# TrackieWay-OSS/TrackieLLM

Hardware: AMD Instinct MI355X
Metric: cortex cycles/sec (frame+1s audio+128 tok) (higher is better)
Workload: dtype int8 x q4_K/q6_K (i32 acc, f32 scales); 1 GPU; configs[3] fused cycle: YOLOv8n 640x640 frame (preprocess+network+NMS) + 1 s PCM (VAD + Whisper-tiny.en log-mel/encoder/16 forced decoder steps) + Mistral-7B Q4_K_M 64-token prefill and 128-token greedy decode, 3 concurrent HIP streams; concurrent_cycles_per_gpu=768, decode_groups=3, rows_per_llm_pass=256, layers=32, parallelism=replicas x1

## Files before the change

### include/tk/tk_mi355x_ext.h

```cpp
#ifndef TK_MI355X_EXT_H
#define TK_MI355X_EXT_H

#include "tk_types.h"

#ifdef __cplusplus
extern "C" {
#endif

typedef struct {
    int32_t n_layer, d_model, n_head, n_kv_head, head_dim, d_ff, vocab;
    float rms_eps, rope_theta;
    int32_t ks_qkv, ks_o, ks_gateup, ks_down, ks_out;
} tk_mi355x_llm_hparams_t;

typedef struct tk_mi355x_llm_model_s tk_mi355x_llm_model_t;
typedef struct tk_mi355x_llm_session_s tk_mi355x_llm_session_t;

TK_API const char* tk_mi355x_version(void);
TK_API int tk_mi355x_device_count(void);
TK_API void tk_mi355x_set_default_device(int device);
TK_API int tk_mi355x_get_default_device(void);

TK_API TK_NODISCARD tk_error_code_t tk_mi355x_llm_model_create(tk_mi355x_llm_model_t** out, const tk_mi355x_llm_hparams_t* hp, int device);
TK_API TK_NODISCARD tk_error_code_t tk_mi355x_llm_model_fill_synthetic(tk_mi355x_llm_model_t* m, uint64_t seed);
// ... 137 lines not shown

TK_API TK_NODISCARD tk_error_code_t tk_mi355x_llm_time_attention(tk_mi355x_llm_session_t* s, int nrows, int ctx, int iters, float* avg_ms,
                                                                 double* kv_bytes);

TK_API int tk_mi355x_device_cu_count(int device);
TK_API TK_NODISCARD tk_error_code_t tk_mi355x_attention_plan(int device, int nrows, int n_head, int n_kv_head, int head_dim, int max_ctx, int fused, int32_t out[4]);
TK_API TK_NODISCARD tk_error_code_t tk_mi355x_attention_plan_at(int device, int nrows, int n_head, int n_kv_head, int head_dim, int max_ctx, int fused,
                                                                int top_position, int32_t out[4]);
TK_API TK_NODISCARD tk_error_code_t tk_mi355x_attention_plan_verify(int device, int nrows, int n_head, int n_kv_head, int head_dim, int max_ctx,
                                                                    int top_position, int32_t out[4]);

TK_API TK_NODISCARD tk_error_code_t tk_mi355x_grammar_check(const char* gbnf, const char* text, int32_t* n_accepted, int32_t* complete);
TK_API TK_NODISCARD tk_error_code_t tk_mi355x_grammar_next_bytes(const char* gbnf, const char* prefix, uint8_t allowed[256], int32_t* complete);
struct tk_llm_runner_s;
TK_API const char* tk_mi355x_llm_runner_tool_call_text(struct tk_llm_runner_s* runner);

TK_API TK_NODISCARD tk_error_code_t tk_mi355x_gemm_pair(int device, int M, int N, int K, const float* a, const float* w, const float* bias,
                                                        const float* residual, int act, int f16, float* c_staged, float* c_tiled);

typedef struct {
    int32_t M, N, K, lda, ldb, ldc, ldr, b_kn, act;
    float alpha;
    int32_t batch, batch_inner;
    int64_t sA, sB, sC, sR, sA2, sB2, sC2, sR2;
    int32_t b_f16;
    int32_t im_C, im_H, im_W, im_ldx, im_kw, im_stride, im_pad, im_Ho, im_Wo;
    int32_t fast;
    int32_t a_offset, b_offset;
    int32_t kernel;
    const float* a; const void* b; const float* bias; const float* residual; float* c;
    int64_t n_a, n_b, n_bias, n_residual, n_c;
} tk_mi355x_gemm_probe_t;
TK_API TK_NODISCARD tk_error_code_t tk_mi355x_gemm_probe(int device, tk_mi355x_gemm_probe_t* p);

TK_API TK_NODISCARD tk_error_code_t tk_mi355x_attention_h3_probe(int device, int B, int nh, int Tq, int Tk, int64_t q_bstride, int64_t kv_bstride, int d, float scale,
                                                                 const float* q, const float* k, const float* v, int64_t n_q, int64_t n_kv, float* out);

enum { TK_MI355X_PICK_ARGMAX = 0, TK_MI355X_PICK_ARGMAX_ROWS = 1, TK_MI355X_PICK_ROWS = 2, TK_MI355X_PICK_ROWS_FILTERED = 3 };
typedef struct {
    int32_t kind, rows, cols, ld;
    const float* logits;
    int64_t n_logits;
    const uint32_t* masks;
    const int32_t* allow_row;
    int32_t n_masks, hist_stride;
    tk_mi355x_sampling_t* samp;
    int32_t *tok, *pos, *nsteps, *hist;
    int64_t n_hist;
    float temperature;
    uint32_t counter0;
    uint64_t seed;
    float* logprob;
    const uint8_t* suppress;
    int32_t* state;
    int32_t beg, eot, tid0, reserved;
} tk_mi355x_token_pick_probe_t;
TK_API TK_NODISCARD tk_error_code_t tk_mi355x_token_pick_probe(int device, tk_mi355x_token_pick_probe_t* p);

TK_API TK_NODISCARD tk_error_code_t tk_mi355x_logit_adjust_probe(int device, int32_t rows, int32_t cols, float* logits, int64_t n_logits,
                                                                 const tk_mi355x_logit_adjust_t* adjust);

TK_API TK_NODISCARD tk_error_code_t tk_mi355x_lang_pick_probe(int device, int32_t rows, int32_t cols, int32_t ld, const float* logits, int64_t n_logits, int32_t tok0,
                                                              int32_t n_lang, const int32_t* auto_row, int32_t* slot, int32_t* ids, float* probs);

enum {
    TK_MI355X_STEP_EMBED = 0, TK_MI355X_STEP_RMSNORM = 1, TK_MI355X_STEP_RESIDUAL_FOLD = 2, TK_MI355X_STEP_SWIGLU = 3, TK_MI355X_STEP_QUANT = 4,
// ... 111 lines not shown
```

### trackiellm_amd/csrc/hal/tk_rocm_hal.hip

```cpp
#include <hip/hip_runtime.h>
#include <math.h>
#include <stdlib.h>

#include <vector>

#include "../common/tk_exact_math.h"
#include "../common/tk_lang_pick.h"
#include "tk/tk_mi355x_ext.h"

#include "../vision/tk_vision_engine.h"
#include "../vision/tk_depth_engine.h"
#include "../audio/tk_audio_engine.h"
#include "tk/tk_rocm_hal.h"
#include "../nn/tk_gemm_tiled.h"
#include "../nn/tk_nn_kernels.h"
#include "../llm/tk_llm_kernels.h"

struct tk_gpu_buffer_s {
    void* dptr;
    size_t size;
};

struct tk_rocm_dispatcher_s {
    int device;
    hipStream_t compute, h2d, d2h;
    hipEvent_t ev_upload, ev_compute;
};

__global__ void k_postprocess_depth(tk_postprocess_depth_params_t p) {
    const size_t n = (size_t)p.width * p.height;
    for (size_t i = (size_t)blockIdx.x * blockDim.x + threadIdx.x; i < n; i += (size_t)gridDim.x * blockDim.x)
        p.d_metric_depth_map[i] = p.d_raw_depth_map[i] * p.scale + p.shift;
}

__global__ void k_depth_to_points(tk_depth_to_points_params_t p) {
    const size_t n = (size_t)p.width * p.height;
    for (size_t i = (size_t)blockIdx.x * blockDim.x + threadIdx.x; i < n; i += (size_t)gridDim.x * blockDim.x) {
        const float d = p.d_metric_depth_map[i];
        tk_float3 o = {0.0f, 0.0f, 0.0f};
        if (d > 0.0f) {
            const float u = (float)(i % p.width), v = (float)(i / p.width);
            o.x = tk_divf((u - p.cx) * d, p.fx);
            o.y = tk_divf((v - p.cy) * d, p.fy);
            o.z = d;
        }
        p.d_point_cloud[i] = o;
    }
// ... 135 lines not shown
    return ok ? TK_SUCCESS : TK_ERROR_GPU_ROCM_ERROR;
}

struct ProbeReach { int64_t a, b, c, r; };
static bool probe_reach(const tk_mi355x_gemm_probe_t& p, ProbeReach& o) {
    const int64_t cap = (int64_t)1 << 28;
    auto dim = [&](int64_t v) { return v >= 1 && v <= cap; };
    auto str = [&](int64_t v) { return v >= 0 && v <= cap; };
    if (!dim(p.M) || !dim(p.N) || !dim(p.K) || !dim(p.ldb) || !dim(p.ldc) || p.ldc < p.N || p.act < 0 || p.act > 3) return false;
    if (p.batch < 1 || p.batch > 4096 || p.batch_inner < 0 || p.batch_inner > p.batch || (p.batch_inner > 0 && p.batch % p.batch_inner)) return false;
    if ((p.b_kn != 0 && p.b_kn != 1) || (p.b_f16 != 0 && p.b_f16 != 1) || p.a_offset < 0 || p.a_offset > 64 || p.b_offset < 0 || p.b_offset > 64) return false;
    const int64_t st[8] = {p.sA, p.sB, p.sC, p.sR, p.sA2, p.sB2, p.sC2, p.sR2};
    for (int64_t v : st) if (!str(v)) return false;
    if (p.residual && (!dim(p.ldr) || p.ldr < p.N)) return false;
    const int64_t zi = p.batch_inner > 0 ? p.batch_inner - 1 : p.batch - 1, zo = p.batch_inner > 0 ? p.batch / p.batch_inner - 1 : 0;
    auto last = [&](int64_t s1, int64_t s2) { return zi * s1 + (p.batch_inner > 0 ? zo * s2 : 0); };
    if (p.im_C > 0) {
        if (!dim(p.im_H) || !dim(p.im_W) || !dim(p.im_ldx) || p.im_ldx < p.im_C || !dim(p.im_kw) || !dim(p.im_stride) || p.im_pad < 0 || p.im_pad > cap ||
            !dim(p.im_Ho) || !dim(p.im_Wo) || p.batch != 1 || p.K % ((int64_t)p.im_C * p.im_kw))
            return false;
        const int64_t images = ((int64_t)p.M - 1) / ((int64_t)p.im_Ho * p.im_Wo) + 1;
        if (images > cap / p.im_H / p.im_W) return false;
        o.a = (images * p.im_H * p.im_W - 1) * p.im_ldx + p.im_C - 1;
    } else {
        if (p.im_C < 0 || !dim(p.lda)) return false;
        o.a = last(p.sA, p.sA2) + ((int64_t)p.M - 1) * p.lda + p.K - 1;
    }
    o.b = last(p.sB, p.sB2) + (p.b_kn ? ((int64_t)p.K - 1) * p.ldb + p.N - 1 : ((int64_t)p.N - 1) * p.ldb + p.K - 1);
    o.c = last(p.sC, p.sC2) + ((int64_t)p.M - 1) * p.ldc + p.N - 1;
    o.r = p.residual ? last(p.sR, p.sR2) + ((int64_t)p.M - 1) * p.ldr + p.N - 1 : -1;
    return true;
}

tk_error_code_t tk_mi355x_gemm_probe(int device, tk_mi355x_gemm_probe_t* p) {
    if (!p) return TK_ERROR_INVALID_ARGUMENT;
    p->kernel = TK_GEMM_REFUSED;
    ProbeReach reach;
    if (!p->a || !p->b || !p->c || !probe_reach(*p, reach)) return TK_ERROR_INVALID_ARGUMENT;
    if (p->n_a < 1 || p->n_b < 1 || p->n_c < 1 || reach.a >= p->n_a || reach.b >= p->n_b || reach.c >= p->n_c) return TK_ERROR_INVALID_ARGUMENT;
    if (p->bias ? p->n_bias < p->N : p->n_bias != 0) return TK_ERROR_INVALID_ARGUMENT;
    if (p->residual ? reach.r >= p->n_residual : p->n_residual != 0) return TK_ERROR_INVALID_ARGUMENT;
    const size_t eb = p->b_f16 ? 2 : 4;
    TkGemm g{};
    g.M = p->M; g.N = p->N; g.K = p->K; g.lda = p->lda; g.ldb = p->ldb; g.ldc = p->ldc; g.ldr = p->ldr; g.b_kn = p->b_kn; g.act = p->act; g.alpha = p->alpha;
    g.batch = p->batch; g.sA = p->sA; g.sB = p->sB; g.sC = p->sC; g.sR = p->sR;
    g.batch_inner = p->batch_inner; g.sA2 = p->sA2; g.sB2 = p->sB2; g.sC2 = p->sC2; g.sR2 = p->sR2;
    g.b_f16 = p->b_f16; g.fast = p->fast;
    g.im_C = p->im_C; g.im_H = p->im_H; g.im_W = p->im_W; g.im_ldx = p->im_ldx; g.im_kw = p->im_kw; g.im_stride = p->im_stride; g.im_pad = p->im_pad;
    g.im_Ho = p->im_Ho; g.im_Wo = p->im_Wo;
    if (device < 0) {
        g.A = (const float*)(uintptr_t)256 + p->a_offset;
        g.B = (const float*)((uintptr_t)256 + (size_t)p->b_offset * eb);
        p->kernel = tk_gemm_kernel_of(g);
        return p->kernel < 0 ? TK_ERROR_INVALID_ARGUMENT : TK_SUCCESS;
    }
    int n = 0;
    if (hipGetDeviceCount(&n) != hipSuccess || n <= 0) return TK_ERROR_GPU_DEVICE_NOT_FOUND;
    if (device >= n || hipSetDevice(device) != hipSuccess) return TK_ERROR_INVALID_ARGUMENT;
    if (!tk_nn_prepare_device()) return TK_ERROR_GPU_ROCM_ERROR;
    float *da = nullptr, *dbias = nullptr, *dr = nullptr, *dc = nullptr;
    uint8_t* db = nullptr;
    const size_t ba = ((size_t)p->n_a + p->a_offset) * 4, bb = ((size_t)p->n_b + p->b_offset) * eb;
    bool ok = hipMalloc((void**)&da, ba) == hipSuccess && hipMalloc((void**)&db, bb) == hipSuccess && hipMalloc((void**)&dc, (size_t)p->n_c * 4) == hipSuccess &&
              (!p->bias || hipMalloc((void**)&dbias, (size_t)p->n_bias * 4) == hipSuccess) &&
              (!p->residual || hipMalloc((void**)&dr, (size_t)p->n_residual * 4) == hipSuccess);
    ok = ok && hipMemcpy(da + p->a_offset, p->a, (size_t)p->n_a * 4, hipMemcpyHostToDevice) == hipSuccess &&
         hipMemcpy(db + (size_t)p->b_offset * eb, p->b, (size_t)p->n_b * eb, hipMemcpyHostToDevice) == hipSuccess &&
         hipMemcpy(dc, p->c, (size_t)p->n_c * 4, hipMemcpyHostToDevice) == hipSuccess &&
         (!p->bias || hipMemcpy(dbias, p->bias, (size_t)p->n_bias * 4, hipMemcpyHostToDevice) == hipSuccess) &&
         (!p->residual || hipMemcpy(dr, p->residual, (size_t)p->n_residual * 4, hipMemcpyHostToDevice) == hipSuccess);
    tk_error_code_t rc = ok ? TK_SUCCESS : TK_ERROR_GPU_ROCM_ERROR;
    if (ok) {
        g.A = da + p->a_offset; g.B = (const float*)(db + (size_t)p->b_offset * eb); g.C = dc; g.bias = dbias; g.residual = dr;
        p->kernel = tk_gemm_kernel_of(g);
        if (!tk_launch_gemm(g, nullptr)) rc = TK_ERROR_INVALID_ARGUMENT;
        else if (hipGetLastError() != hipSuccess) rc = TK_ERROR_GPU_KERNEL_LAUNCH;
        else if (hipDeviceSynchronize() != hipSuccess || hipMemcpy(p->c, dc, (size_t)p->n_c * 4, hipMemcpyDeviceToHost) != hipSuccess) rc = TK_ERROR_GPU_ROCM_ERROR;
    }
    void* ptrs[] = {da, db, dbias, dr, dc};
    for (void* q : ptrs) if (q) (void)hipFree(q);
    return rc;
}

tk_error_code_t tk_mi355x_attention_h3_probe(int device, int B, int nh, int Tq, int Tk, int64_t q_bstride, int64_t kv_bstride, int d, float scale, const float* q,
                                             const float* k, const float* v, int64_t n_q, int64_t n_kv, float* out) {
    const int64_t cap = (int64_t)1 << 28;
    if (!q || !k || !v || !out || B < 1 || B > 4096 || nh < 1 || nh > 4096 || Tq < 1 || Tq > cap || Tk < 1 || Tk > cap || d < 1 || d > cap || q_bstride < 0 ||
        q_bstride > cap || kv_bstride < 0 || kv_bstride > cap)
        return TK_ERROR_INVALID_ARGUMENT;
    if (d != nh * 64 || (q_bstride & 3) || (kv_bstride & 3)) return TK_ERROR_INVALID_ARGUMENT;
    if ((B - 1) * q_bstride + (int64_t)Tq * d > n_q || (B - 1) * kv_bstride + (int64_t)Tk * d > n_kv) return TK_ERROR_INVALID_ARGUMENT;
    if (B > 1 && (q_bstride < (int64_t)Tq * d || kv_bstride < (int64_t)Tk * d)) return TK_ERROR_INVALID_ARGUMENT;
    int n = 0;
    if (hipGetDeviceCount(&n) != hipSuccess || n <= 0) return TK_ERROR_GPU_DEVICE_NOT_FOUND;
    if (device < 0 || device >= n || hipSetDevice(device) != hipSuccess) return TK_ERROR_INVALID_ARGUMENT;
    float *dq = nullptr, *dk = nullptr, *dv = nullptr, *dout = nullptr;
    bool ok = hipMalloc((void**)&dq, (size_t)n_q * 4) == hipSuccess && hipMalloc((void**)&dk, (size_t)n_kv * 4) == hipSuccess &&
              hipMalloc((void**)&dv, (size_t)n_kv * 4) == hipSuccess && hipMalloc((void**)&dout, (size_t)n_q * 4) == hipSuccess;
    ok = ok && hipMemcpy(dq, q, (size_t)n_q * 4, hipMemcpyHostToDevice) == hipSuccess && hipMemcpy(dk, k, (size_t)n_kv * 4, hipMemcpyHostToDevice) == hipSuccess &&
         hipMemcpy(dv, v, (size_t)n_kv * 4, hipMemcpyHostToDevice) == hipSuccess && hipMemcpy(dout, out, (size_t)n_q * 4, hipMemcpyHostToDevice) == hipSuccess;
    tk_error_code_t rc = ok ? TK_SUCCESS : TK_ERROR_GPU_ROCM_ERROR;
    if (ok) {
        if (!tk_launch_attention_h3(dq, dk, dv, dout, B, nh, Tq, Tk, q_bstride, kv_bstride, d, scale, nullptr)) rc = TK_ERROR_INVALID_ARGUMENT;
        else if (hipGetLastError() != hipSuccess) rc = TK_ERROR_GPU_KERNEL_LAUNCH;
        else if (hipDeviceSynchronize() != hipSuccess || hipMemcpy(out, dout, (size_t)n_q * 4, hipMemcpyDeviceToHost) != hipSuccess) rc = TK_ERROR_GPU_ROCM_ERROR;
    }
    void* ptrs[] = {dq, dk, dv, dout};
    for (void* p : ptrs) if (p) (void)hipFree(p);
    return rc;
}

static bool pick_probe_ok(const tk_mi355x_token_pick_probe_t& p) {
    static_assert(sizeof(tk_mi355x_sampling_t) == sizeof(TkSampleRow), "the public sampling state is the kernels' TkSampleRow");
    const bool llm = p.kind == TK_MI355X_PICK_ARGMAX;
    if (p.kind < TK_MI355X_PICK_ARGMAX || p.kind > TK_MI355X_PICK_ROWS_FILTERED || !p.logits) return false;
// ... 763 lines not shown
```

### trackiellm_amd/csrc/nn/tk_nn_kernels.hip

```cpp
#include "tk_nn_kernels.h"

#include <atomic>
#include <mutex>

#include "../common/tk_exact_math.h"
#include "../common/tk_lang_pick.h"
#include "../common/tk_sample_device.h"

typedef float v16f __attribute__((ext_vector_type(16)));

#define BM 64
#define BN 64
#define BK 32
#define LDS_LD (BK + 1)

__device__ __forceinline__ float ldb1(const float* B, int f16, int64_t i) {
    return f16 ? (float)((const _Float16*)B)[i] : B[i];
}
__device__ __forceinline__ void ldb4(const float* B, int f16, int64_t i, float* out) {
    if (f16) {
        const uint2 t = *(const uint2*)((const _Float16*)B + i);
        const _Float16* h = (const _Float16*)&t;
        out[0] = (float)h[0]; out[1] = (float)h[1]; out[2] = (float)h[2]; out[3] = (float)h[3];
    } else {
        const float4 t = *(const float4*)(B + i);
        out[0] = t.x; out[1] = t.y; out[2] = t.z; out[3] = t.w;
    }
}

__device__ __forceinline__ float apply_act(float v, int act) {
    switch (act) {
        case TK_ACT_SILU: return tk_siluf(v);
        case TK_ACT_GELU: return tk_geluf(v);
        case TK_ACT_SIGMOID: return tk_sigmoidf(v);
        default: return v;
    }
}

struct ImRow { int64_t pix0; int iy0, ix0; bool ok; };
struct ImCol { int c, kx, ky; };
__device__ __forceinline__ ImRow im_row(const TkGemm& g, int m) {
    ImRow r;
// ... 39 lines not shown
        else {
#pragma unroll
            for (int i = 0; i < 4; ++i) if (k + i < g.K) out[i] = p[i];
        }
    }
}
template <int PATH>
__device__ __forceinline__ void load_b4_nk(const TkGemm& g, const float* B, bool b_vec, int n, int k, float out[4]) {
    if (PATH != 0) { ld4_if(n < g.N && k < g.K, B + (int64_t)n * g.ldb + k, out); return; }
    out[0] = out[1] = out[2] = out[3] = 0.0f;
    if (n < g.N) {
        const int64_t p = (int64_t)n * g.ldb + k;
        if (b_vec && k + 3 < g.K) ldb4(B, g.b_f16, p, out);
        else {
#pragma unroll
            for (int i = 0; i < 4; ++i) if (k + i < g.K) out[i] = ldb1(B, g.b_f16, p + i);
        }
    }
}
template <int PATH>
__device__ __forceinline__ void load_b4_kn(const TkGemm& g, const float* B, bool b_vec, int k, int n, float out[4]) {
    if (PATH != 0) { ld4_if(k < g.K && n < g.N, B + (int64_t)k * g.ldb + n, out); return; }
    out[0] = out[1] = out[2] = out[3] = 0.0f;
    if (k < g.K) {
        const int64_t p = (int64_t)k * g.ldb + n;
        if (b_vec && n + 3 < g.N) ldb4(B, g.b_f16, p, out);
        else {
#pragma unroll
            for (int i = 0; i < 4; ++i) if (n + i < g.N) out[i] = ldb1(B, g.b_f16, p + i);
        }
    }
}

__device__ __forceinline__ float fast_sigmoidf(float x) { return __builtin_amdgcn_rcpf(1.0f + __builtin_amdgcn_exp2f(x * -1.4426950408889634f)); }
__device__ __forceinline__ float fast_geluf(float x) {
    const float inner = 0.797884560802865356f * (x + 0.044715f * ((x * x) * x));
    const float th = 1.0f - 2.0f * __builtin_amdgcn_rcpf(__builtin_amdgcn_exp2f(inner * 2.8853900817779268f) + 1.0f);
    return (0.5f * x) * (1.0f + th);
}

template <bool FASTACT = false>
__device__ __forceinline__ void store_tile(const TkGemm& g, const v16f& acc, float* C, const float* R, int m_base, int n, int lane) {
    if (n >= g.N) return;
    const float bias = g.bias ? g.bias[n] : 0.0f;
    const float alpha = g.alpha;
    float v[16];
#pragma unroll
    for (int r = 0; r < 16; ++r) v[r] = acc[r];
    if (alpha != 1.0f) {
#pragma unroll
        for (int r = 0; r < 16; ++r) v[r] = v[r] * alpha;
    }
#pragma unroll
    for (int r = 0; r < 16; ++r) v[r] = v[r] + bias;
    if (g.act == TK_ACT_SILU) {
#pragma unroll
        for (int r = 0; r < 16; ++r) v[r] = FASTACT ? v[r] * fast_sigmoidf(v[r]) : tk_siluf(v[r]);
    } else if (g.act == TK_ACT_GELU) {
#pragma unroll
        for (int r = 0; r < 16; ++r) v[r] = FASTACT ? fast_geluf(v[r]) : tk_geluf(v[r]);
    } else if (g.act == TK_ACT_SIGMOID) {
#pragma unroll
        for (int r = 0; r < 16; ++r) v[r] = FASTACT ? fast_sigmoidf(v[r]) : tk_sigmoidf(v[r]);
    }
    const int mb = m_base + 4 * (lane >> 5);
    float* cp = C + (int64_t)mb * g.ldc + n;
    if (m_base + 32 <= g.M) {
        if (R) {
            const float* rp = R + (int64_t)mb * g.ldr + n;
#pragma unroll
            for (int r = 0; r < 16; ++r) v[r] = v[r] + rp[(int64_t)((r & 3) + 8 * (r >> 2)) * g.ldr];
        }
#pragma unroll
        for (int r = 0; r < 16; ++r) cp[(int64_t)((r & 3) + 8 * (r >> 2)) * g.ldc] = v[r];
        return;
    }
    if (R) {
        const float* rp = R + (int64_t)mb * g.ldr + n;
#pragma unroll
        for (int r = 0; r < 16; ++r) {
            const int dm = (r & 3) + 8 * (r >> 2);
            if (mb + dm < g.M) v[r] = v[r] + rp[(int64_t)dm * g.ldr];
        }
    }
#pragma unroll
    for (int r = 0; r < 16; ++r) {
        const int dm = (r & 3) + 8 * (r >> 2);
        if (mb + dm < g.M) cp[(int64_t)dm * g.ldc] = v[r];
    }
}

__device__ __forceinline__ void batch_offsets(const TkGemm& g, int z, int64_t& oA, int64_t& oB, int64_t& oC, int64_t& oR) {
    if (g.batch_inner > 0) {
        const int zo = z / g.batch_inner, zi = z % g.batch_inner;
        oA = zo * g.sA2 + zi * g.sA; oB = zo * g.sB2 + zi * g.sB; oC = zo * g.sC2 + zi * g.sC; oR = zo * g.sR2 + zi * g.sR;
    } else {
        oA = (int64_t)z * g.sA; oB = (int64_t)z * g.sB; oC = (int64_t)z * g.sC; oR = (int64_t)z * g.sR;
// ... 531 lines not shown
#pragma unroll
        for (int rr = 0; rr < 4; ++rr) {
            float4 w;
            w.x = (o_hh[t][4 * rr + 0] + o_hx[t][4 * rr + 0] * (1.0f / H3_SCALE)) * inv;
            w.y = (o_hh[t][4 * rr + 1] + o_hx[t][4 * rr + 1] * (1.0f / H3_SCALE)) * inv;
            w.z = (o_hh[t][4 * rr + 2] + o_hx[t][4 * rr + 2] * (1.0f / H3_SCALE)) * inv;
            w.w = (o_hh[t][4 * rr + 3] + o_hx[t][4 * rr + 3] * (1.0f / H3_SCALE)) * inv;
            *(float4*)(op + t * 32 + 4 * g + 8 * rr) = w;
        }
}

bool tk_launch_attention_h3(const float* q, const float* k, const float* v, float* out, int B, int nh, int Tq, int Tk, int64_t q_bstride, int64_t kv_bstride, int d,
                            float scale, hipStream_t s) {
    if (d != nh * 64 || (d & 3) || Tq < 1 || Tk < 1 || ((((uintptr_t)q) | ((uintptr_t)k) | ((uintptr_t)v) | ((uintptr_t)out)) & 15) || (q_bstride & 3) || (kv_bstride & 3)) return false;
    hipLaunchKernelGGL(k_attention_h3, dim3((Tq + 127) / 128, nh, B), dim3(256), 0, s, q, k, v, out, Tq, Tk, q_bstride, kv_bstride, d, scale);
    return true;
}

static std::atomic<bool> g_big_opted[64];
static std::mutex g_big_mu;
bool tk_nn_prepare_device() {
    const size_t lds = (size_t)2 * (LBM + LBN) * LDS_LD * sizeof(float);
    int dev = 0;
    if (hipGetDevice(&dev) != hipSuccess || dev < 0 || dev >= 64) return false;
    if (g_big_opted[dev].load(std::memory_order_acquire)) return true;
    std::lock_guard<std::mutex> lk(g_big_mu);
    const void* fns[4] = {(const void*)k_gemm_f32_big<false, 0>, (const void*)k_gemm_f32_big<false, 1>, (const void*)k_gemm_f32_big<false, 2>,
                          (const void*)k_gemm_f32_big<true, 1>};
    for (const void* f : fns)
        if (hipFuncSetAttribute(f, hipFuncAttributeMaxDynamicSharedMemorySize, (int)lds) != hipSuccess) return false;
    const void* h3[2] = {(const void*)k_gemm_h3_big<false>, (const void*)k_gemm_h3_big<true>};
    for (const void* f : h3)
        if (hipFuncSetAttribute(f, hipFuncAttributeMaxDynamicSharedMemorySize, (int)H3_BIG_LDS) != hipSuccess) return false;
    g_big_opted[dev].store(true, std::memory_order_release);
    return true;
}

static bool tk_gemm_fast(const TkGemm& g) {
    auto m4 = [](int64_t v) { return (v & 3) == 0; };
    if (g.b_f16 || !m4(g.K) || !m4(g.ldb) || (((uintptr_t)g.B) & 15)) return false;
    if (g.im_C == 0 && (!m4(g.lda) || (((uintptr_t)g.A) & 15))) return false;
    if (g.b_kn && !m4(g.N)) return false;
    if (g.batch > 1 && (!m4(g.sA) || !m4(g.sB))) return false;
    if (g.batch_inner > 0 && (!m4(g.sA2) || !m4(g.sB2))) return false;
    return true;
}

int tk_gemm_kernel_of(const TkGemm& g) {
    if (g.M < 1 || g.N < 1 || g.K < 0) return TK_GEMM_REFUSED;
    const int nz = g.batch > 0 ? g.batch : 1;
    const bool im = g.im_C > 0;
    const int path = tk_gemm_fast(g) ? (g.b_kn ? 2 : 1) : 0;
    if (im && (path == 0 || g.b_kn || (g.im_C & 3) || (g.im_ldx & 3) || (((uintptr_t)g.A) & 15) || g.im_kw < 1 || g.K % (g.im_C * g.im_kw) || g.im_stride < 1 || g.im_Ho < 1 ||
               g.im_Wo < 1))
        return TK_GEMM_REFUSED;
    const int lp = im ? 1 : path;
    const int nt = (g.N + 31) / 32;
    const bool fast = g.fast != 0 && !g.b_kn && (im || path == 1);
    if (fast && g.N >= 96) return TK_GEMM_CODE(TK_GEMM_H3_BIG, im, 1, 0);
    if (fast && nz == 1 && g.batch_inner == 0) return TK_GEMM_CODE(TK_GEMM_H3_TALL, im, 1, nt);
    if (g.M >= 256 && g.N >= 96) return TK_GEMM_CODE(TK_GEMM_F32_BIG, im, lp, 0);
    if (g.N < 96 && g.M >= 4 * NBM && !g.b_kn && !g.b_f16 && nz == 1 && g.batch_inner == 0)
        return TK_GEMM_CODE(TK_GEMM_F32_TALL, im, lp, nt);
    return TK_GEMM_CODE(TK_GEMM_F32, im, lp, 0);
}

// ... 659 lines not shown
```

### trackiellm_amd/csrc/vision/tk_vision_engine.hip

```cpp
#include "tk_vision_engine.h"
#include "tk_onnx_weights.h"

#include <stdio.h>
#include <string.h>

#include "../common/tk_box_attr.h"
#include "../nn/tk_nn_kernels.h"

static inline hipError_t tk_create_perception_stream(hipStream_t* s) {
    int lo = 0, hi = 0;
    if (hipDeviceGetStreamPriorityRange(&lo, &hi) != hipSuccess) return hipStreamCreateWithFlags(s, hipStreamNonBlocking);
    return hipStreamCreateWithPriority(s, hipStreamNonBlocking, hi);
}

#define HIPQ(expr)                                                                              \
    do {                                                                                        \
        hipError_t e__ = (expr);                                                                \
        if (e__ != hipSuccess) {                                                                \
            char b__[256];                                                                      \
            snprintf(b__, sizeof b__, "%s failed: %s (%s:%d)", #expr, hipGetErrorString(e__), __FILE__, __LINE__); \
            error = b__;                                                                        \
            return false;                                                                       \
        }                                                                                       \
    } while (0)

__global__ void k_preprocess(TkPreprocessArgs a) {
    const uint32_t ox = blockIdx.x * blockDim.x + threadIdx.x, oy = blockIdx.y * blockDim.y + threadIdx.y;
    if (ox >= a.out_w || oy >= a.out_h) return;
    const float x_ratio = tk_divf((float)a.in_w - 1.0f, (float)a.out_w);
    const float y_ratio = tk_divf((float)a.in_h - 1.0f, (float)a.out_h);
    const float gx = x_ratio * (float)ox, gy = y_ratio * (float)oy;
    const int x = (int)gx, y = (int)gy;
    const float xd = gx - (float)x, yd = gy - (float)y;
    const int x1 = x + 1 < (int)a.in_w ? x + 1 : x, y1 = y + 1 < (int)a.in_h ? y + 1 : y;
    const uint8_t* r0 = a.src + (size_t)y * a.in_stride;
    const uint8_t* r1 = a.src + (size_t)y1 * a.in_stride;
    const size_t np = (size_t)a.out_w * a.out_h, pix = (size_t)oy * a.out_w + ox;
#pragma unroll
    for (int c = 0; c < 3; ++c) {
// ... 115 lines not shown
    if (n == specs.size() + 1 && ox.convs.back().cout == 1 && ox.convs.back().cin == TK_YOLO_REG_MAX && ox.convs.back().kh == 1) --n;
    if (n != specs.size())
        return yolo_generic_graph(path, this, "the ONNX graph has " + std::to_string(ox.convs.size()) + " Conv nodes, YOLOv8n has " + std::to_string(specs.size()) + " (+ DFL)");
    for (size_t i = 0; i < n; ++i) {
        const TkConvSpec& s = specs[i];
        const TkOnnxConv& c = ox.convs[i];
        if (c.cout != s.cout || c.cin != s.cin || c.kh != s.k || c.kw != s.k)
            return yolo_generic_graph(path, this, "Conv " + std::to_string(i) + " is [" + std::to_string(c.cout) + "][" + std::to_string(c.cin) + "][" + std::to_string(c.kh) + "][" +
                                                      std::to_string(c.kw) + "], the YOLOv8n graph expects [" + std::to_string(s.cout) + "][" + std::to_string(s.cin) + "][" +
                                                      std::to_string(s.k) + "][" + std::to_string(s.k) + "]");
    }
    std::vector<float> hw;
    for (size_t i = 0; i < n; ++i) {
        const TkConvSpec& s = specs[i];
        const TkOnnxConv& c = ox.convs[i];
        if (c.cout != s.cout || c.cin != s.cin || c.kh != s.k || c.kw != s.k) {
            error = "Conv " + std::to_string(i) + " does not match the YOLOv8n graph";
            return false;
        }
        hw.resize(c.w.size());
        for (int o = 0; o < s.cout; ++o)
            for (int ci = 0; ci < s.cin; ++ci)
                for (int k = 0; k < s.k * s.k; ++k) hw[((size_t)o * s.k * s.k + k) * s.cin + ci] = c.w[((size_t)o * s.cin + ci) * s.k * s.k + k];
        if (!set_layer((int)i, hw.data(), c.b.data())) return false;
    }
    return true;
}


struct TkGpuOps {
    TkDetector* d;
    hipStream_t s;
    bool refused = false;
    TkT alloc(int B, int H, int W, int C) {
        TkT t;
        t.B = B; t.H = H; t.W = W; t.C = C; t.ld = C;
        size_t n = ((size_t)B * H * W * C + 63) & ~(size_t)63;
        t.p = d->arena + d->arena_used;
        d->arena_used += n;
        return t;
    }
    void conv(const TkT& x, int idx, const TkT& y, const TkT* res) {
        const TkConvSpec& sp = d->model->specs[idx];
        TkGemm g{};
        g.M = y.B * y.H * y.W; g.N = sp.cout; g.K = sp.k * sp.k * sp.cin;
        if (sp.k == 1 && sp.s == 1) { g.A = x.p; g.lda = x.ld; }
        else if (tk_gemm_im2col_ok(x.p, x.C, x.ld, d->model->w[idx])) {
            g.A = x.p; g.lda = 0;
            g.im_C = x.C; g.im_H = x.H; g.im_W = x.W; g.im_ldx = x.ld; g.im_kw = sp.k; g.im_stride = sp.s; g.im_pad = sp.k / 2;
            g.im_Ho = y.H; g.im_Wo = y.W;
        } else if (!res && tk_launch_conv_stem(x.p, x.B, x.H, x.W, x.C, x.ld, d->model->w[idx], d->model->b[idx], sp.act ? TK_ACT_SILU : TK_ACT_NONE, sp.cout, sp.k,
                                               sp.s, sp.k / 2, y.p, y.ld, s)) {
            return;
        } else {
            if (!tk_launch_im2col(x.p, x.B, x.H, x.W, x.C, x.ld, sp.k, sp.k, sp.s, sp.k / 2, d->col, s)) refused = true;
            g.A = d->col; g.lda = g.K;
        }
        g.B = d->model->w[idx]; g.ldb = g.K; g.b_kn = 0;
        g.C = y.p; g.ldc = y.ld;
        g.bias = d->model->b[idx];
        g.residual = res ? res->p : nullptr; g.ldr = res ? res->ld : 0;
        g.act = sp.act ? TK_ACT_SILU : TK_ACT_NONE;
        g.alpha = 1.0f; g.batch = 1;
        g.fast = d->fast ? 1 : 0;
        if (!tk_launch_gemm(g, s)) refused = true;
    }
    void maxpool5(const TkT& x, const TkT& y) { if (!tk_launch_maxpool5(x.p, x.B, x.H, x.W, x.C, x.ld, y.p, y.ld, s)) refused = true; }
    void upsample2x(const TkT& x, const TkT& y) { if (!tk_launch_upsample2x(x.p, x.B, x.H, x.W, x.C, x.ld, y.p, y.ld, s)) refused = true; }
    void copy(const TkT& x, const TkT& y) { if (!tk_launch_copy_cols(x.p, x.B * x.H * x.W, x.C, x.ld, y.p, y.ld, s)) refused = true; }
};

struct TkSizeOps {
    const std::vector<TkConvSpec>* specs;
    size_t used = 0, col = 0;
    TkT alloc(int B, int H, int W, int C) {
        TkT t;
        t.B = B; t.H = H; t.W = W; t.C = C; t.ld = C;
        used += ((size_t)B * H * W * C + 63) & ~(size_t)63;
        return t;
    }
    void conv(const TkT&, int idx, const TkT& y, const TkT*) {
        const TkConvSpec& sp = (*specs)[idx];
        if (!(sp.k == 1 && sp.s == 1)) { size_t n = (size_t)y.B * y.H * y.W * sp.k * sp.k * sp.cin; col = n > col ? n : col; }
    }
    void maxpool5(const TkT&, const TkT&) {}
    void upsample2x(const TkT&, const TkT&) {}
    void copy(const TkT&, const TkT&) {}
};


__global__ void k_yolo_decode(TkT h0, TkT h1, TkT h2, int nc, int n_anchors, float conf, tk_yolo_cand_t* cand) {
    const int a = blockIdx.x * blockDim.x + threadIdx.x, b = blockIdx.y;
    if (a >= n_anchors) return;
    const int n0 = h0.H * h0.W, n1 = h1.H * h1.W;
    const TkT* h;
    int local;
    float stride;
// ... 114 lines not shown
}

bool tk_launch_yolo_decode_out(const float* out, int nc, int n_anchors, float conf, tk_yolo_cand_t* cand, hipStream_t s) {
    if (nc < 1 || n_anchors < 1) return false;
    hipLaunchKernelGGL(k_yolo_decode_out, dim3((n_anchors + 255) / 256), dim3(256), 0, s, out, nc, n_anchors, conf, cand);
    return true;
}

bool tk_launch_yolo_post(const tk_yolo_cand_t* cand, int n_anchors, int B, float iou, int32_t* order, int32_t* n_cand, uint64_t* mask, TkDetection* kept,
                         int32_t* n_kept, hipStream_t s) {
    if (B < 1 || B > 65535 || n_anchors < 1) return false;
    hipLaunchKernelGGL(k_yolo_rank, dim3((n_anchors + 255) / 256, B), dim3(256), 0, s, cand, n_anchors, order, n_cand);
    hipLaunchKernelGGL(k_yolo_mask, dim3(TK_YOLO_MAX_CAND / 64 / 8, TK_YOLO_MAX_CAND / 8, B), dim3(8, 8), 0, s, cand, n_anchors, order, n_cand, iou, mask);
    hipLaunchKernelGGL(k_yolo_scan, dim3(B), dim3(64), 0, s, cand, n_anchors, order, n_cand, mask, kept, n_kept);
    return true;
}


TkDetector::~TkDetector() {
    if (model) (void)hipSetDevice(model->device);
    if (stream) (void)hipStreamSynchronize(stream);
    void* ptrs[] = {frame_dev, arena, col, input, cand, order, n_cand, mask, kept, n_kept, attr_dev};
    for (void* p : ptrs) if (p) (void)hipFree(p);
    if (exec) exec->unload();
    if (stream) (void)hipStreamDestroy(stream);
}

bool TkDetector::init(TkYoloModel* m, int w, int h, int mb) {
    model = m; in_w = w; in_h = h; max_batch = mb;
    if (!m || w <= 0 || h <= 0 || (w % 32) || (h % 32)) { error = "detector input must be a positive multiple of 32"; return false; }
    if (mb < 1 || mb > 256) { error = "max_batch must be in [1,256]"; return false; }
    HIPQ(hipSetDevice(m->device));
    HIPQ(tk_create_perception_stream(&stream));
    n_anchors = (h / 8) * (w / 8) + (h / 16) * (w / 16) + (h / 32) * (w / 32);
    if (m->generic) {
        exec.reset(new TkOnnxExec());
        if (!exec->load(m->onnx_path.c_str(), m->device, stream, (size_t)320 * h * w + (1u << 22))) { error = "detector graph: " + exec->error; return false; }
    } else {
        TkSizeOps so{&m->specs};
        TkT x = so.alloc(mb, h, w, 3);
        so.used = 0;
        TkT o[3];
        TkYoloV8n<TkSizeOps>::forward(so, x, o, m->nc);
        arena_floats = so.used + 1024;
        col_floats = so.col + 1024;
        HIPQ(hipMalloc((void**)&arena, arena_floats * 4));
        HIPQ(hipMalloc((void**)&col, col_floats * 4));
    }
    HIPQ(hipMalloc((void**)&input, (size_t)mb * h * w * 3 * 4));
    HIPQ(hipMalloc((void**)&cand, (size_t)mb * n_anchors * sizeof(tk_yolo_cand_t)));
    HIPQ(hipMalloc((void**)&order, (size_t)mb * TK_YOLO_MAX_CAND * 4));
    HIPQ(hipMalloc((void**)&n_cand, (size_t)mb * 4));
    HIPQ(hipMalloc((void**)&mask, (size_t)mb * TK_YOLO_MAX_CAND * (TK_YOLO_MAX_CAND / 64) * 8));
    HIPQ(hipMalloc((void**)&kept, (size_t)mb * TK_OBJECT_DETECTOR_MAX_DETECTIONS * sizeof(TkDetection)));
    HIPQ(hipMalloc((void**)&n_kept, (size_t)mb * 4));
    return true;
}

bool TkDetector::run_graph(int B, float* host_out) {
    for (int b = 0; b < B; ++b) {
        exec->begin();
        TkOnnxExec::Val in;
        in.d = input + (size_t)b * 3 * in_h * in_w;
        in.shape = {1, 3, in_h, in_w};
        exec->bind(model->graph_in, in);
        if (!exec->run()) { error = "detector graph: " + exec->error; return false; }
// ... 191 lines not shown
```

Baseline: 187.3 cycles/s.

## Add direct 3x3 convolution kernel with LDS input patch for small-channel YOLO layers

Adds a direct 3x3 convolution kernel that stages an input spatial patch plus halo in LDS and streams double-buffered weight tiles into fp32 MFMA, avoiding implicit im2col address generation in the tiled GEMM. The YOLOv8n conv path routes stride-1 3x3 convs with at most 16 input channels and at most 96 outputs to it, with an environment variable to disable. The shared epilogue is factored into a header, and a probe entry point is added for testing. This only affects a few early vision layers, which are a small slice of a cycle dominated by the LLM.

Result: no change. 187.3 cycles/s, median of 2 (+0.0%).

```diff
diff --git a/include/tk/tk_mi355x_ext.h b/include/tk/tk_mi355x_ext.h
--- a/include/tk/tk_mi355x_ext.h
+++ b/include/tk/tk_mi355x_ext.h
@@ -193,6 +193,7 @@
     int64_t n_a, n_b, n_bias, n_residual, n_c;
 } tk_mi355x_gemm_probe_t;
 TK_API TK_NODISCARD tk_error_code_t tk_mi355x_gemm_probe(int device, tk_mi355x_gemm_probe_t* p);
+TK_API TK_NODISCARD tk_error_code_t tk_mi355x_conv3x3_probe(int device, tk_mi355x_gemm_probe_t* p);
 
 TK_API TK_NODISCARD tk_error_code_t tk_mi355x_attention_h3_probe(int device, int B, int nh, int Tq, int Tk, int64_t q_bstride, int64_t kv_bstride, int d, float scale,
                                                                  const float* q, const float* k, const float* v, int64_t n_q, int64_t n_kv, float* out);
diff --git a/trackiellm_amd/csrc/hal/tk_rocm_hal.hip b/trackiellm_amd/csrc/hal/tk_rocm_hal.hip
--- a/trackiellm_amd/csrc/hal/tk_rocm_hal.hip
+++ b/trackiellm_amd/csrc/hal/tk_rocm_hal.hip
@@ -13,6 +13,7 @@
 #include "../audio/tk_audio_engine.h"
 #include "tk/tk_rocm_hal.h"
 #include "../nn/tk_gemm_tiled.h"
+#include "../nn/tk_conv_direct.h"
 #include "../nn/tk_nn_kernels.h"
 #include "../llm/tk_llm_kernels.h"
 
@@ -214,9 +215,9 @@
     return true;
 }
 
-tk_error_code_t tk_mi355x_gemm_probe(int device, tk_mi355x_gemm_probe_t* p) {
+static tk_error_code_t gemm_probe_run(int device, tk_mi355x_gemm_probe_t* p, bool direct) {
     if (!p) return TK_ERROR_INVALID_ARGUMENT;
-    p->kernel = TK_GEMM_REFUSED;
+    p->kernel = direct ? 0 : TK_GEMM_REFUSED;
     ProbeReach reach;
     if (!p->a || !p->b || !p->c || !probe_reach(*p, reach)) return TK_ERROR_INVALID_ARGUMENT;
     if (p->n_a < 1 || p->n_b < 1 || p->n_c < 1 || reach.a >= p->n_a || reach.b >= p->n_b || reach.c >= p->n_c) return TK_ERROR_INVALID_ARGUMENT;
@@ -233,6 +234,7 @@
     if (device < 0) {
         g.A = (const float*)(uintptr_t)256 + p->a_offset;
         g.B = (const float*)((uintptr_t)256 + (size_t)p->b_offset * eb);
+        if (direct) { p->kernel = tk_conv3x3_direct_ok(g) ? 1 : 0; return TK_SUCCESS; }
         p->kernel = tk_gemm_kernel_of(g);
         return p->kernel < 0 ? TK_ERROR_INVALID_ARGUMENT : TK_SUCCESS;
     }
@@ -254,8 +256,10 @@
     tk_error_code_t rc = ok ? TK_SUCCESS : TK_ERROR_GPU_ROCM_ERROR;
     if (ok) {
         g.A = da + p->a_offset; g.B = (const float*)(db + (size_t)p->b_offset * eb); g.C = dc; g.bias = dbias; g.residual = dr;
-        p->kernel = tk_gemm_kernel_of(g);
-        if (!tk_launch_gemm(g, nullptr)) rc = TK_ERROR_INVALID_ARGUMENT;
+        if (direct) p->kernel = tk_launch_conv3x3_direct(g, nullptr) ? 1 : 0;
+        else p->kernel = tk_gemm_kernel_of(g);
+        if (direct && p->kernel == 0) rc = TK_SUCCESS;
+        else if (!direct && !tk_launch_gemm(g, nullptr)) rc = TK_ERROR_INVALID_ARGUMENT;
         else if (hipGetLastError() != hipSuccess) rc = TK_ERROR_GPU_KERNEL_LAUNCH;
         else if (hipDeviceSynchronize() != hipSuccess || hipMemcpy(p->c, dc, (size_t)p->n_c * 4, hipMemcpyDeviceToHost) != hipSuccess) rc = TK_ERROR_GPU_ROCM_ERROR;
     }
@@ -263,6 +267,9 @@
     for (void* q : ptrs) if (q) (void)hipFree(q);
     return rc;
 }
+
+tk_error_code_t tk_mi355x_gemm_probe(int device, tk_mi355x_gemm_probe_t* p) { return gemm_probe_run(device, p, false); }
+tk_error_code_t tk_mi355x_conv3x3_probe(int device, tk_mi355x_gemm_probe_t* p) { return gemm_probe_run(device, p, true); }
 
 tk_error_code_t tk_mi355x_attention_h3_probe(int device, int B, int nh, int Tq, int Tk, int64_t q_bstride, int64_t kv_bstride, int d, float scale, const float* q,
                                              const float* k, const float* v, int64_t n_q, int64_t n_kv, float* out) {
diff --git a/trackiellm_amd/csrc/nn/tk_conv_direct.h b/trackiellm_amd/csrc/nn/tk_conv_direct.h
--- /dev/null
+++ b/trackiellm_amd/csrc/nn/tk_conv_direct.h
@@ -0,0 +1,17 @@
+#ifndef TK_CONV_DIRECT_H
+#define TK_CONV_DIRECT_H
+
+#include <hip/hip_runtime.h>
+#include <stddef.h>
+
+#include "../common/tk_gemm_desc.h"
+
+#define TK_CONV_DIRECT_LDS_BYTES (80 * 1024)
+
+bool tk_conv3x3_direct_ok(const TkGemm& g);
+bool tk_conv3x3_direct_admit(const TkGemm& g);
+size_t tk_conv3x3_direct_lds_bytes(const TkGemm& g);
+bool tk_launch_conv3x3_direct(const TkGemm& g, hipStream_t s);
+bool tk_conv_direct_prepare_device();
+
+#endif
diff --git a/trackiellm_amd/csrc/nn/tk_conv_direct.hip b/trackiellm_amd/csrc/nn/tk_conv_direct.hip
--- /dev/null
+++ b/trackiellm_amd/csrc/nn/tk_conv_direct.hip
@@ -0,0 +1,215 @@
+#include "tk_conv_direct.h"
+
+#include "tk_gemm_epilogue.h"
+#include "tk_nn_kernels.h"
+
+#define CD_TH 8
+#define CD_TW 16
+#define CD_BK 32
+#define CD_BLD (CD_BK + 1)
+
+struct CdLayout { int PH, PW, CP, RP, NT; size_t floats; };
+static bool cd_layout(int C, int N, int stride, CdLayout& L) {
+    if (C < 4 || C > 4096 || N < 1 || N > 96 || (stride != 1 && stride != 2)) return false;
+    L.PH = (CD_TH - 1) * stride + 3;
+    L.PW = (CD_TW - 1) * stride + 3;
+    L.CP = C + 1;
+    L.RP = L.PW * L.CP;
+    L.RP += (16 - (L.RP & 31)) & 31;
+    L.NT = (N + 31) / 32;
+    L.floats = (size_t)L.PH * L.RP + (size_t)2 * L.NT * 32 * CD_BLD;
+    return true;
+}
+
+template <int NT, int S>
+__global__ __launch_bounds__(256) void k_conv3x3_direct(TkGemm g, int CP, int RP) {
+    extern __shared__ __attribute__((aligned(16))) float cd_lds[];
+    constexpr int PH = (CD_TH - 1) * S + 3, PW = (CD_TW - 1) * S + 3;
+    float* patch = cd_lds;
+    float* Bs = cd_lds + PH * RP;
+    const int tid = threadIdx.x, lane = tid & 63, wave = tid >> 6;
+    const int C = g.im_C, H = g.im_H, W = g.im_W, K = g.K;
+    const int b = blockIdx.z, oy0 = blockIdx.y * CD_TH, ox0 = blockIdx.x * CD_TW;
+    const float* Wt = g.B;
+
+    float rb[NT][4];
+    auto gload_b = [&](int k0) {
+        const int k = k0 + (tid & 7) * 4;
+#pragma unroll
+        for (int t = 0; t < NT; ++t) {
+            const int n = (tid >> 3) + 32 * t;
+            float4 v = make_float4(0.0f, 0.0f, 0.0f, 0.0f);
+            if (n < g.N && k < K) v = *(const float4*)(Wt + (int64_t)n * g.ldb + k);
+            rb[t][0] = v.x; rb[t][1] = v.y; rb[t][2] = v.z; rb[t][3] = v.w;
+        }
+    };
+    auto lstore_b = [&](int buf) {
+        float* bs = Bs + buf * (NT * 32 * CD_BLD) + (tid >> 3) * CD_BLD + (tid & 7) * 4;
+#pragma unroll
+        for (int t = 0; t < NT; ++t)
+#pragma unroll
+            for (int i = 0; i < 4; ++i) bs[t * 32 * CD_BLD + i] = rb[t][i];
+    };
+    gload_b(0);
+
+    {
+        const int c4n = C >> 2, total = PH * PW * c4n;
+        const int iy0 = oy0 * S - 1, ix0 = ox0 * S - 1;
+        const float* X = g.A + (int64_t)b * H * W * g.im_ldx;
+        for (int e0 = tid; e0 < total; e0 += 1024) {
+            float4 v[4];
+            int off[4];
+#pragma unroll
+            for (int u = 0; u < 4; ++u) {
+                const int e = e0 + 256 * u;
+                const int pix = e / c4n, cg = e - pix * c4n, py = pix / PW, px = pix - py * PW;
+                const int iy = iy0 + py, ix = ix0 + px;
+                off[u] = e < total ? py * RP + px * CP + cg * 4 : -1;
+                v[u] = make_float4(0.0f, 0.0f, 0.0f, 0.0f);
+                if (e < total && iy >= 0 && iy < H && ix >= 0 && ix < W) v[u] = *(const float4*)(X + ((int64_t)iy * W + ix) * g.im_ldx + cg * 4);
+            }
+#pragma unroll
+            for (int u = 0; u < 4; ++u)
+                if (off[u] >= 0) {
+                    float* p = patch + off[u];
+                    p[0] = v[u].x; p[1] = v[u].y; p[2] = v[u].z; p[3] = v[u].w;
+                }
+        }
+    }
+    lstore_b(0);
+    __syncthreads();
+
+    v16f acc[NT];
+#pragma unroll
+    for (int t = 0; t < NT; ++t)
+#pragma unroll
+        for (int i = 0; i < 16; ++i) acc[t][i] = 0.0f;
+    const int i32 = lane & 31, h = lane >> 5;
+    const float* ap = patch + ((2 * wave + (i32 >> 4)) * S) * RP + ((i32 & 15) * S) * CP + h;
+    const float* bp0 = Bs + i32 * CD_BLD + h;
+    int c = 0, kx = 0, toff = 0;
+    auto advance = [&]() {
+        c += 2;
+        const bool tap = c == C;
+        c = tap ? 0 : c;
+        toff += tap ? CP : 0;
+        kx += tap ? 1 : 0;
+        const bool row = kx == 3;
+        kx = row ? 0 : kx;
+        toff += row ? RP - 3 * CP : 0;
+    };
+    int buf = 0;
+    for (int k0 = 0; k0 < K; k0 += CD_BK) {
+        const bool more = k0 + CD_BK < K;
+        if (more) gload_b(k0 + CD_BK);
+        const float* bp = bp0 + buf * (NT * 32 * CD_BLD);
+        if (k0 + CD_BK <= K) {
+            int aoff[CD_BK / 2];
+#pragma unroll
+            for (int j = 0; j < CD_BK / 2; ++j) { aoff[j] = toff + c; advance(); }
+#pragma unroll
+            for (int j = 0; j < CD_BK / 2; ++j) {
+                const float av = ap[aoff[j]];
+#pragma unroll
+                for (int t = 0; t < NT; ++t) acc[t] = __builtin_amdgcn_mfma_f32_32x32x2f32(av, bp[t * 32 * CD_BLD + 2 * j], acc[t], 0, 0, 0);
+            }
+        } else {
+            for (int kk = 0; k0 + kk < K; kk += 2) {
+                const float av = ap[toff + c];
+#pragma unroll
+                for (int t = 0; t < NT; ++t) acc[t] = __builtin_amdgcn_mfma_f32_32x32x2f32(av, bp[t * 32 * CD_BLD + kk], acc[t], 0, 0, 0);
+                advance();
+            }
+        }
+        if (more) lstore_b(buf ^ 1);
+        __syncthreads();
+        buf ^= 1;
+    }
+
+    const float* R = g.residual;
+    const int Ho = g.im_Ho, Wo = g.im_Wo;
+    const int oy = oy0 + 2 * wave, ox = ox0 + 4 * h;
+    const int64_t m0 = ((int64_t)b * Ho + oy) * Wo + ox;
+    const int64_t m_in = ((int64_t)b * Ho + oy0) * Wo + ox0;
+    const bool full = oy0 + CD_TH <= Ho && ox0 + CD_TW <= Wo;
+#pragma unroll
+    for (int t = 0; t < NT; ++t) {
+        const int n = 32 * t + i32;
+        if (n >= g.N) continue;
+        float v[16];
+        tile_epilogue(g, acc[t], n, v);
+        if (R) {
+            float rv[16];
+#pragma unroll
+            for (int r = 0; r < 16; ++r) {
+                const int dx = (r & 3) + 8 * ((r >> 2) & 1);
+                const bool in = full || (oy + (r >> 3) < Ho && ox + dx < Wo);
+                const int64_t m = in ? m0 + (r >> 3) * Wo + dx : m_in;
+                rv[r] = R[m * g.ldr + n];
+            }
+#pragma unroll
+            for (int r = 0; r < 16; ++r) v[r] = v[r] + rv[r];
+        }
+        float* cp = g.C + m0 * g.ldc + n;
+#pragma unroll
+        for (int r = 0; r < 16; ++r) {
+            const int dx = (r & 3) + 8 * ((r >> 2) & 1);
+            if (full || (oy + (r >> 3) < Ho && ox + dx < Wo)) cp[(int64_t)((r >> 3) * Wo + dx) * g.ldc] = v[r];
+        }
+    }
+}
+
+size_t tk_conv3x3_direct_lds_bytes(const TkGemm& g) {
+    CdLayout L;
+    if (g.im_C < 1 || !cd_layout(g.im_C, g.N, g.im_stride, L)) return 0;
+    return L.floats * sizeof(float);
+}
+
+bool tk_conv3x3_direct_ok(const TkGemm& g) {
+    if (g.im_C < 4 || (g.im_C & 3) || (g.im_ldx & 3) || g.im_ldx < g.im_C || g.im_kw != 3 || g.im_pad != 1 || g.fast || g.b_kn || g.b_f16) return false;
+    if (g.im_stride != 1 && g.im_stride != 2) return false;
+    if (g.N < 1 || g.N > 96 || g.K != 9 * g.im_C || g.ldb < g.K || (g.ldb & 3) || g.ldc < g.N || (g.residual && g.ldr < g.N)) return false;
+    if (g.batch > 1 || g.batch_inner != 0) return false;
+    if (((((uintptr_t)g.A) | ((uintptr_t)g.B)) & 15) != 0) return false;
+    if (g.im_H < 1 || g.im_W < 1 || g.im_Ho != (g.im_H - 1) / g.im_stride + 1 || g.im_Wo != (g.im_W - 1) / g.im_stride + 1) return false;
+    const int64_t per = (int64_t)g.im_Ho * g.im_Wo;
+    if (g.M < 1 || g.M % per || g.M / per > 65535 || g.im_Ho > 65535 * CD_TH || g.im_Wo > 65535 * CD_TW) return false;
+    const size_t lds = tk_conv3x3_direct_lds_bytes(g);
+    return lds > 0 && lds <= TK_CONV_DIRECT_LDS_BYTES;
+}
+
+bool tk_conv3x3_direct_admit(const TkGemm& g) { return tk_conv3x3_direct_ok(g) && g.im_stride == 1 && g.im_C <= 16; }
+
+template <int S>
+static const void* cd_kernel(int nt) {
+    switch (nt) {
+        case 1: return (const void*)k_conv3x3_direct<1, S>;
+        case 2: return (const void*)k_conv3x3_direct<2, S>;
+        default: return (const void*)k_conv3x3_direct<3, S>;
+    }
+}
+
+bool tk_conv_direct_prepare_device() {
+    for (int nt = 1; nt <= 3; ++nt) {
+        if (hipFuncSetAttribute(cd_kernel<1>(nt), hipFuncAttributeMaxDynamicSharedMemorySize, TK_CONV_DIRECT_LDS_BYTES) != hipSuccess) return false;
+        if (hipFuncSetAttribute(cd_kernel<2>(nt), hipFuncAttributeMaxDynamicSharedMemorySize, TK_CONV_DIRECT_LDS_BYTES) != hipSuccess) return false;
+    }
+    return true;
+}
+
+bool tk_launch_conv3x3_direct(const TkGemm& g, hipStream_t s) {
+    if (!tk_conv3x3_direct_ok(g)) return false;
+    CdLayout L;
+    cd_layout(g.im_C, g.N, g.im_stride, L);
+    const size_t lds = L.floats * sizeof(float);
+    if (lds > 64 * 1024 && !tk_nn_prepare_device()) return false;
+    const dim3 grid((g.im_Wo + CD_TW - 1) / CD_TW, (g.im_Ho + CD_TH - 1) / CD_TH, (unsigned)(g.M / ((int64_t)g.im_Ho * g.im_Wo)));
+#define CD_LAUNCH(NT, S) hipLaunchKernelGGL((k_conv3x3_direct<NT, S>), grid, dim3(256), lds, s, g, L.CP, L.RP)
+    if (g.im_stride == 1) {
+        if (L.NT == 1) CD_LAUNCH(1, 1); else if (L.NT == 2) CD_LAUNCH(2, 1); else CD_LAUNCH(3, 1);
+    } else {
+        if (L.NT == 1) CD_LAUNCH(1, 2); else if (L.NT == 2) CD_LAUNCH(2, 2); else CD_LAUNCH(3, 2);
+    }
+#undef CD_LAUNCH
+    return true;
+}
diff --git a/trackiellm_amd/csrc/nn/tk_gemm_epilogue.h b/trackiellm_amd/csrc/nn/tk_gemm_epilogue.h
--- /dev/null
+++ b/trackiellm_amd/csrc/nn/tk_gemm_epilogue.h
@@ -0,0 +1,42 @@
+#ifndef TK_GEMM_EPILOGUE_H
+#define TK_GEMM_EPILOGUE_H
+
+#include <hip/hip_runtime.h>
+
+#include "../common/tk_exact_math.h"
+#include "../common/tk_gemm_desc.h"
+
+typedef float v16f __attribute__((ext_vector_type(16)));
+
+__device__ __forceinline__ float fast_sigmoidf(float x) { return __builtin_amdgcn_rcpf(1.0f + __builtin_amdgcn_exp2f(x * -1.4426950408889634f)); }
+__device__ __forceinline__ float fast_geluf(float x) {
+    const float inner = 0.797884560802865356f * (x + 0.044715f * ((x * x) * x));
+    const float th = 1.0f - 2.0f * __builtin_amdgcn_rcpf(__builtin_amdgcn_exp2f(inner * 2.8853900817779268f) + 1.0f);
+    return (0.5f * x) * (1.0f + th);
+}
+
+template <bool FASTACT = false>
+__device__ __forceinline__ void tile_epilogue(const TkGemm& g, const v16f& acc, int n, float v[16]) {
+    const float bias = g.bias ? g.bias[n] : 0.0f;
+    const float alpha = g.alpha;
+#pragma unroll
+    for (int r = 0; r < 16; ++r) v[r] = acc[r];
+    if (alpha != 1.0f) {
+#pragma unroll
+        for (int r = 0; r < 16; ++r) v[r] = v[r] * alpha;
+    }
+#pragma unroll
+    for (int r = 0; r < 16; ++r) v[r] = v[r] + bias;
+    if (g.act == TK_ACT_SILU) {
+#pragma unroll
+        for (int r = 0; r < 16; ++r) v[r] = FASTACT ? v[r] * fast_sigmoidf(v[r]) : tk_siluf(v[r]);
+    } else if (g.act == TK_ACT_GELU) {
+#pragma unroll
+        for (int r = 0; r < 16; ++r) v[r] = FASTACT ? fast_geluf(v[r]) : tk_geluf(v[r]);
+    } else if (g.act == TK_ACT_SIGMOID) {
+#pragma unroll
+        for (int r = 0; r < 16; ++r) v[r] = FASTACT ? fast_sigmoidf(v[r]) : tk_sigmoidf(v[r]);
+    }
+}
+
+#endif
diff --git a/trackiellm_amd/csrc/nn/tk_nn_kernels.hip b/trackiellm_amd/csrc/nn/tk_nn_kernels.hip
--- a/trackiellm_amd/csrc/nn/tk_nn_kernels.hip
+++ b/trackiellm_amd/csrc/nn/tk_nn_kernels.hip
@@ -6,8 +6,8 @@
 #include "../common/tk_exact_math.h"
 #include "../common/tk_lang_pick.h"
 #include "../common/tk_sample_device.h"
-
-typedef float v16f __attribute__((ext_vector_type(16)));
+#include "tk_conv_direct.h"
+#include "tk_gemm_epilogue.h"
 
 #define BM 64
 #define BN 64
@@ -113,37 +113,11 @@
     }
 }
 
-__device__ __forceinline__ float fast_sigmoidf(float x) { return __builtin_amdgcn_rcpf(1.0f + __builtin_amdgcn_exp2f(x * -1.4426950408889634f)); }
-__device__ __forceinline__ float fast_geluf(float x) {
-    const float inner = 0.797884560802865356f * (x + 0.044715f * ((x * x) * x));
-    const float th = 1.0f - 2.0f * __builtin_amdgcn_rcpf(__builtin_amdgcn_exp2f(inner * 2.8853900817779268f) + 1.0f);
-    return (0.5f * x) * (1.0f + th);
-}
-
 template <bool FASTACT = false>
 __device__ __forceinline__ void store_tile(const TkGemm& g, const v16f& acc, float* C, const float* R, int m_base, int n, int lane) {
     if (n >= g.N) return;
-    const float bias = g.bias ? g.bias[n] : 0.0f;
-    const float alpha = g.alpha;
     float v[16];
-#pragma unroll
-    for (int r = 0; r < 16; ++r) v[r] = acc[r];
-    if (alpha != 1.0f) {
-#pragma unroll
-        for (int r = 0; r < 16; ++r) v[r] = v[r] * alpha;
-    }
-#pragma unroll
-    for (int r = 0; r < 16; ++r) v[r] = v[r] + bias;
-    if (g.act == TK_ACT_SILU) {
-#pragma unroll
-        for (int r = 0; r < 16; ++r) v[r] = FASTACT ? v[r] * fast_sigmoidf(v[r]) : tk_siluf(v[r]);
-    } else if (g.act == TK_ACT_GELU) {
-#pragma unroll
-        for (int r = 0; r < 16; ++r) v[r] = FASTACT ? fast_geluf(v[r]) : tk_geluf(v[r]);
-    } else if (g.act == TK_ACT_SIGMOID) {
-#pragma unroll
-        for (int r = 0; r < 16; ++r) v[r] = FASTACT ? fast_sigmoidf(v[r]) : tk_sigmoidf(v[r]);
-    }
+    tile_epilogue<FASTACT>(g, acc, n, v);
     const int mb = m_base + 4 * (lane >> 5);
     float* cp = C + (int64_t)mb * g.ldc + n;
     if (m_base + 32 <= g.M) {
@@ -741,6 +715,7 @@
     const void* h3[2] = {(const void*)k_gemm_h3_big<false>, (const void*)k_gemm_h3_big<true>};
     for (const void* f : h3)
         if (hipFuncSetAttribute(f, hipFuncAttributeMaxDynamicSharedMemorySize, (int)H3_BIG_LDS) != hipSuccess) return false;
+    if (!tk_conv_direct_prepare_device()) return false;
     g_big_opted[dev].store(true, std::memory_order_release);
     return true;
 }
diff --git a/trackiellm_amd/csrc/vision/tk_vision_engine.hip b/trackiellm_amd/csrc/vision/tk_vision_engine.hip
--- a/trackiellm_amd/csrc/vision/tk_vision_engine.hip
+++ b/trackiellm_amd/csrc/vision/tk_vision_engine.hip
@@ -2,9 +2,11 @@
 #include "tk_onnx_weights.h"
 
 #include <stdio.h>
+#include <stdlib.h>
 #include <string.h>
 
 #include "../common/tk_box_attr.h"
+#include "../nn/tk_conv_direct.h"
 #include "../nn/tk_nn_kernels.h"
 
 static inline hipError_t tk_create_perception_stream(hipStream_t* s) {
@@ -186,6 +188,7 @@
     TkDetector* d;
     hipStream_t s;
     bool refused = false;
+    bool direct = [] { const char* e = getenv("TK_MI355X_NO_DIRECT_CONV"); return !(e && e[0] == '1'); }();
     TkT alloc(int B, int H, int W, int C) {
         TkT t;
         t.B = B; t.H = H; t.W = W; t.C = C; t.ld = C;
@@ -217,6 +220,7 @@
         g.act = sp.act ? TK_ACT_SILU : TK_ACT_NONE;
         g.alpha = 1.0f; g.batch = 1;
         g.fast = d->fast ? 1 : 0;
+        if (g.im_C > 0 && direct && tk_conv3x3_direct_admit(g) && tk_launch_conv3x3_direct(g, s)) return;
         if (!tk_launch_gemm(g, s)) refused = true;
     }
     void maxpool5(const TkT& x, const TkT& y) { if (!tk_launch_maxpool5(x.p, x.B, x.H, x.W, x.C, x.ld, y.p, y.ld, s)) refused = true; }
@@ -397,6 +401,7 @@
     if (mb < 1 || mb > 256) { error = "max_batch must be in [1,256]"; return false; }
     HIPQ(hipSetDevice(m->device));
     HIPQ(tk_create_perception_stream(&stream));
+    if (!tk_nn_prepare_device()) { error = "tk_nn_prepare_device failed"; return false; }
     n_anchors = (h / 8) * (w / 8) + (h / 16) * (w / 16) + (h / 32) * (w / 32);
     if (m->generic) {
         exec.reset(new TkOnnxExec());
```
